# gregorgebhardt/gym-kilobots

Measured on AMD Instinct MI355X. Metric: kilobot-steps/sec, higher is better.
Workload: dtype f32

## Files before the change

### gym_kilobots_amd/csrc/kb_common.h

```cpp
#pragma once
#include <hip/hip_runtime.h>

#include <cmath>
#include <cstdio>
#include <cstring>
#include <type_traits>

#include "kilobots_hip.h"
#include "kb_launch.h"
#include "kb_exact.h"

namespace kb {

constexpr float B2_PI = 3.14159265359f;
constexpr float B2_LINEAR_SLOP = 0.005f;
constexpr float B2_POLYGON_RADIUS = 2.0f * B2_LINEAR_SLOP;
constexpr float B2_BAUMGARTE = 0.2f;
constexpr float B2_MAX_LINEAR_CORRECTION = 0.2f;
constexpr float B2_MAX_TRANSLATION = 2.0f;
constexpr float B2_MAX_TRANSLATION_SQ = B2_MAX_TRANSLATION * B2_MAX_TRANSLATION;
constexpr float B2_MAX_ROTATION = 0.5f * B2_PI;
constexpr float B2_MAX_ROTATION_SQ = B2_MAX_ROTATION * B2_MAX_ROTATION;
constexpr float B2_EPSILON = 1.19209290e-07f;
constexpr float B2_TOI_BAUMGARTE = 0.75f;
constexpr int B2_MAX_SUBSTEPS = 8;
constexpr float B2_TIME_TO_SLEEP = 0.5f;
constexpr float B2_LINEAR_SLEEP_TOL = 0.01f;
constexpr float B2_ANGULAR_SLEEP_TOL = 2.0f / 180.0f * B2_PI;
constexpr float WORLD_SCALE = 25.0f;

constexpr float CELL_SIZE = 0.875f;
constexpr int MAX_CELLS = 8192;

constexpr unsigned KEY_WALL = 0x10000u, KEY_OBJ = 0x20000u;
constexpr int WALL_CODE = 0xFFF0;
constexpr int OBJ_CODE = 0xFFE0;
constexpr int MAXOBJ = KB_MAX_OBJECTS;
constexpr unsigned short EMPTY16 = 0xFFFFu;

#ifndef KB_KREG
#define KB_KREG 2
#endif
constexpr int MAX_BUCKETS = MAX_WAVES * BK_PER_WAVE;
constexpr int GIANT_ISLAND = 256;
constexpr int BIG_ISLAND = 16;
constexpr int KREG = KB_KREG;
#ifndef KB_NSOLVE_DIV
#define KB_NSOLVE_DIV 1
#endif
#ifndef KB_KREG_BINS
#define KB_KREG_BINS (2 * KB_NSOLVE_DIV)
#endif

enum { M_NCON = 0, M_TOTAL = 1, M_ANY = 2, M_STATUS = 3, M_MAXISL = 4, M_PROF = 5, M_XTRA = 6, M_XFILL = 7, M_WCNT = 8, M_WAKE = 32 , M_WFILL = 8 + MAX_WAVES, M_COUNT = 8 + 2 * MAX_WAVES };
static_assert(M_COUNT <= 64, "misc area");

struct Params {
    kb_buffers buf;
    const float *actions;
    const float *light_action;
    int N, NP, NB, M, E, S, gw, gh, ncell, cap, capL, n_substeps, flags, drive_mode, light_type, vel_iters, pos_iters;
    int solver_mode, toi_walls;
    float xmin, ymin, xmax, ymax, inv_cell, r_bot, im_bot, kl_bot, ka_bot, h;
    float light_radius, light_lo[2], light_hi[2], act_lo[2], act_hi[2];
    int lcount, ladim, lkind[KB_MAX_LIGHTS];
    float lradius[KB_MAX_LIGHTS], lmaxv[KB_MAX_LIGHTS];
    float llo[KB_MAX_LIGHTS][2], lhi[KB_MAX_LIGHTS][2], lalo[KB_MAX_LIGHTS][2], lahi[KB_MAX_LIGHTS][2];
    float kl_obj, ka_obj;
    float otab[KB_MAX_OBJECTS][OT_WORDS_C];
    float obody[KB_MAX_OBJECTS][BT_WORDS_C];
    int F;
    float mu_oo, mu_ow;
    int nmc;
    int lds_total;
    int nhead, hmask;
    int allow_sleep;
    float im_mode[5];
    int botlaw_off;
    int islmin_off;
    int sense_s;
    float sense_r2;
    float rr2, rw2, rw_tot;
    float toi_tt;
    float nm_bb, nm_wb;
    float y_bb, y_wb;
    int exact_div;
    const unsigned char *env_mask;
};


__device__ __forceinline__ void kb_sincosf(float xx, float &sn, float &cs) {
    const float DP1 = 0.78515625f, DP2 = 2.4187564849853515625e-4f, DP3 = 3.77489497744594108e-8f;
    const float FOPI = 1.27323954473516f;
    float x = fabsf(xx);
    int j = (int)(FOPI * x);
    float y = (float)j;
    if (j & 1) { j += 1; y += 1.0f; }
    j &= 7;
    float ssign = xx < 0.0f ? -1.0f : 1.0f, csign = 1.0f;
    if (j > 3) { ssign = -ssign; csign = -csign; j -= 4; }
    if (j > 1) csign = -csign;
    x = ((x - y * DP1) - y * DP2) - y * DP3;
    float z = x * x;
    float pc = ((2.443315711809948E-005f * z - 1.388731625493765E-003f) * z + 4.166664568298827E-002f) * z * z
               - 0.5f * z + 1.0f;
    float ps = ((-1.9515295891E-4f * z + 8.3321608736E-3f) * z - 1.6666654611E-1f) * z * x + x;
    if (j == 1 || j == 2) { sn = ssign * pc; cs = csign * ps; }
    else { sn = ssign * ps; cs = csign * pc; }
}

__device__ __forceinline__ void kb_light_circular(float sx, float sy, float lx, float ly, float R,
                                                  float &val, float &gx, float &gy) {
    float dx = -1.0f * (sx - lx), dy = -1.0f * (sy - ly);
    float n = sqrtf(dx * dx + dy * dy);
    float v = 1.0f - n / R;
    v = fmaxf(fminf(v, 1.0f), 0.0f);
    val = v * 255.0f;
    if (n > 0.0f) { dx = dx / n; dy = dy / n; }
    else { dx = 0.0f; dy = 0.0f; }
    if (n > R) { dx *= 0.0f; dy *= 0.0f; }
    gx = dx; gy = dy;
}

__device__ __forceinline__ void kb_light_single_step(const Params &p, const float *la, float h, float &lx, float &ly) {
    float ax = fminf(fmaxf(la[0], p.act_lo[0]), p.act_hi[0]);
    float ay = fminf(fmaxf(la[1], p.act_lo[1]), p.act_hi[1]);
    float nlx = lx + ax * h, nly = ly + ay * h;
    lx = fminf(fmaxf(nlx, p.light_lo[0]), p.light_hi[0]);
    ly = fminf(fmaxf(nly, p.light_lo[1]), p.light_hi[1]);
}
__device__ __forceinline__ void kb_light_general_step(const Params &p, const float *la, float h, float (&glx)[KB_MAX_LIGHTS],
                                                      float (&gly)[KB_MAX_LIGHTS], float (&glvx)[KB_MAX_LIGHTS], float (&glvy)[KB_MAX_LIGHTS]) {
    if (p.light_type == KB_LIGHT_GRADIENT) {
        const float pi = 3.14159265358979323846f;
        float ang = fminf(fmaxf(la[0], -2.0f * pi), 2.0f * pi);
        if (ang < -pi) ang += 2.0f * pi;
        if (ang > pi) ang -= 2.0f * pi;
        glx[0] = ang;
    } else {
#pragma unroll
        for (int i = 0; i < KB_MAX_LIGHTS; ++i) {
            if (i >= p.lcount) break;
            const float ax = fminf(fmaxf(la[2 * i + 0], p.lalo[i][0]), p.lahi[i][0]);
            const float ay = fminf(fmaxf(la[2 * i + 1], p.lalo[i][1]), p.lahi[i][1]);
            float nlx, nly;
            if (p.lkind[i] == KB_LIGHT_MOMENTUM) {
                float mvx = glvx[i] + ax * h, mvy = glvy[i] + ay * h;
                const float nv = sqrtf(mvx * mvx + mvy * mvy);
                if (nv > p.lmaxv[i]) { const float sc = p.lmaxv[i] / nv; mvx *= sc; mvy *= sc; }
                glvx[i] = mvx; glvy[i] = mvy;
                nlx = glx[i] + mvx * h; nly = gly[i] + mvy * h;
            } else {
                nlx = glx[i] + ax * h; nly = gly[i] + ay * h;
            }
            glx[i] = fminf(fmaxf(nlx, p.llo[i][0]), p.lhi[i][0]);
            gly[i] = fminf(fmaxf(nly, p.llo[i][1]), p.lhi[i][1]);
        }
    }
}
__device__ __forceinline__ void kb_light_general_sense(const Params &p, const float (&glx)[KB_MAX_LIGHTS], const float (&gly)[KB_MAX_LIGHTS],
                                                       float sx, float sy, float &val, float &gx, float &gy) {
    if (p.light_type == KB_LIGHT_GRADIENT) {
        float s_, c_;
        kb_sincosf(glx[0], s_, c_);
        val = c_ * sx + s_ * sy; gx = c_; gy = s_;
        return;
    }
    float vsum = 0.0f, vbest = 0.0f, bgx = 0.0f, bgy = 0.0f;
#pragma unroll
    for (int i = 0; i < KB_MAX_LIGHTS; ++i) {
        if (i >= p.lcount) break;
        float v, x, y;
        kb_light_circular(sx, sy, glx[i], gly[i], p.lradius[i], v, x, y);
        vsum = i == 0 ? v : vsum + v;
        if (i == 0 || v > vbest) { vbest = v; bgx = x; bgy = y; }
    }
    val = vsum; gx = bgx; gy = bgy;
}

__device__ __forceinline__ void kb_motor_law(int ml, int mr, float th, float h, float &vx, float &vy, float &w) {
    const float max_lin = 0.01f, max_ang = 0.5f * 3.14159265358979323846f;
    float s, c;
    kb_sincosf(th, s, c);
    if (ml && mr) {
        float lin = (float)(mr + ml) / 510.0f * max_lin;
        vx = (s * lin) * WORLD_SCALE; vy = (c * lin) * WORLD_SCALE;
        w = (float)(mr - ml) / 510.0f * max_ang;
    } else if (mr || ml) {
        float av, lx, ly = -0.009f;
        if (mr) { av = (float)mr / 255.0f * max_ang; lx = -0.013f; }
        else { av = -(float)ml / 255.0f * max_ang; lx = 0.013f; }
        float ds, dc;
        kb_sincosf(av * h, ds, dc);
        float tx = lx - (dc * lx - ds * ly), ty = ly - (ds * lx + dc * ly);
        tx *= WORLD_SCALE; ty *= WORLD_SCALE;
        float wx = c * tx - s * ty, wy = s * tx + c * ty;
        wx = wx / WORLD_SCALE / h; wy = wy / WORLD_SCALE / h;
        vx = wx * WORLD_SCALE; vy = wy * WORLD_SCALE; w = av;
    } else {
        vx = 0.0f; vy = 0.0f; w = 0.0f;
    }
}

__device__ __forceinline__ float kb_clampf(float a, float lo, float hi) { return fmaxf(lo, fminf(a, hi)); }

__device__ __forceinline__ void wave_sync() {
    __builtin_amdgcn_fence(__ATOMIC_RELEASE, "wavefront");
    __builtin_amdgcn_wave_barrier();
    __builtin_amdgcn_fence(__ATOMIC_ACQUIRE, "wavefront");
}

template <bool DS_ATOMIC = false>
__device__ __forceinline__ unsigned lds_load_relaxed(const unsigned *p_) {
    if constexpr (DS_ATOMIC) return atomicOr(const_cast<unsigned *>(p_), 0u);
    else return *reinterpret_cast<const volatile unsigned *>(p_);
}

__device__ __forceinline__ void lds_barrier() {
    asm volatile("s_waitcnt lgkmcnt(0)\n\ts_barrier" ::: "memory");
}

#define KB_DPP(v, ctrl, rows) __builtin_amdgcn_update_dpp(0, (int)(v), ctrl, rows, 0xf, true)
__device__ __forceinline__ unsigned wave_or(unsigned v) {
    v |= (unsigned)KB_DPP(v, 0x111, 0xf);
    v |= (unsigned)KB_DPP(v, 0x112, 0xf);
    v |= (unsigned)KB_DPP(v, 0x114, 0xf);
    v |= (unsigned)KB_DPP(v, 0x118, 0xf);
    v |= (unsigned)KB_DPP(v, 0x142, 0xa);
    v |= (unsigned)KB_DPP(v, 0x143, 0xc);
    return (unsigned)__builtin_amdgcn_readlane((int)v, 63);
}
__device__ __forceinline__ unsigned wave_umax(unsigned v) {
    v = max(v, (unsigned)KB_DPP(v, 0x111, 0xf));
    v = max(v, (unsigned)KB_DPP(v, 0x112, 0xf));
    v = max(v, (unsigned)KB_DPP(v, 0x114, 0xf));
    v = max(v, (unsigned)KB_DPP(v, 0x118, 0xf));
    v = max(v, (unsigned)KB_DPP(v, 0x142, 0xa));
    v = max(v, (unsigned)KB_DPP(v, 0x143, 0xc));
    return (unsigned)__builtin_amdgcn_readlane((int)v, 63);
}
__device__ __forceinline__ unsigned wave_incl_scan(unsigned v) {
// ... 347 lines not shown
```

### gym_kilobots_amd/csrc/kb_step_kernel.h

```cpp
#pragma once
#include <utility>

#include "kb_common.h"
#include "kb_objects.h"

namespace kb {

template <int DRIVE_MODE, int LIGHT_TYPE, bool OBJ, int FN = 0, int TIER = 0, bool POLY = true, bool SENSE = true, bool SLEEP = false>
__global__ void __launch_bounds__(TIER == 1 ? 64 : 64 * KB_MAX_WAVES, (TIER == 1 || TIER == 3) ? 2 : ((TIER == 2 || (FN != 0 && !OBJ)) ? KB_COMPACT_WAVES_PER_SIMD : KB_MIN_WAVES_PER_SIMD)) kb_step_kernel(const Params p) {
    constexpr bool WIDE = TIER == 1 || TIER == 3;
    constexpr bool BINS = !OBJ;
    constexpr int KRX = BINS ? KB_KREG_BINS : KREG;
    constexpr bool PAR_DS = FN != 0 && BINS;
    static_assert(!SLEEP || FN == 0 || !OBJ, "the fixed-size instantiations with objects do not carry the sleep state");
    extern __shared__ __align__(16) unsigned char smem[];
    {
        static_assert(sizeof(Params) >= 6 * 64, "the six lines asked for are kernel arguments");
        const __attribute__((address_space(4))) unsigned *ka_ = (const __attribute__((address_space(4))) unsigned *)__builtin_amdgcn_kernarg_segment_ptr();
        const __attribute__((address_space(1))) unsigned char *m_ = (const __attribute__((address_space(1))) unsigned char *)p.env_mask;
        asm volatile("" : "+s"(m_) : "s"(ka_[0]), "s"(ka_[16]), "s"(ka_[32]), "s"(ka_[48]), "s"(ka_[64]), "s"(ka_[80]));
        if (m_ && !m_[blockIdx.x]) return;
    }
    int e = blockIdx.x;
    int tid = threadIdx.x;
    const int nt = FN ? 64 * KB_MAX_WAVES : (int)blockDim.x;
    int lane = tid & 63, wave = tid >> 6;
    const int wave_s = __builtin_amdgcn_readfirstlane(wave);
    const int nw = nt >> 6;
    const int nsolve = BINS ? (nw >= KB_NSOLVE_DIV ? nw / KB_NSOLVE_DIV : 1) : nw;
    const int N = FN ? FN : p.N, NP = FN ? ((FN + 3) & ~3) : p.NP, S = p.S;
    size_t o = (size_t)e * N;
    size_t wo = (size_t)e * p.cap;
    const float h = p.h;

    const int NB = FN ? ((FN + 3) & ~3) + KB_MAX_OBJECTS + 4 : p.NB;
    const int capL_ = (BINS && FN != 0) ? ldsb::CAPL : p.capL;
    const bool hashed = FN == 0 && p.hmask != 0;
    const int fx = lds::fixed(OBJ || FN != 0, nw), ot_ = lds::objtab(nw);
    float2 *pos = (float2 *)(smem + (BINS ? ldsb::pos() : lds::body32(fx, NB, 0))), *vel = (float2 *)(smem + (BINS ? ldsb::vel(NB) : lds::body32(fx, NB, 2)));
    float2 *start = (float2 *)(smem + lds::body32(fx, NB, 4));
    unsigned *dirCnt = (unsigned *)(smem + (BINS ? ldsb::dircnt(NB) : lds::body32(fx, NB, 6))), *parent = (unsigned *)(smem + (BINS ? ldsb::parent(NB) : lds::body32(fx, NB, 7)));
    unsigned *islCnt = dirCnt;
    unsigned *lPair = (unsigned *)(smem + (BINS ? ldsb::con32(NB, NP, hashed, capL_, 0) : lds::con32(fx, NB, capL_, 0))), *lInfo = (unsigned *)(smem + (BINS ? ldsb::con32(NB, NP, hashed, capL_, 1) : lds::con32(fx, NB, capL_, 1)));
    float *lAcc = (float *)(smem + (BINS ? ldsb::con32(NB, NP, hashed, capL_, 2) : lds::con32(fx, NB, capL_, 2)));
    float *oldAcc = (float *)(smem + (BINS ? ldsb::oldacc(NB, NP, hashed, capL_) : lds::con32(fx, NB, capL_, 3)));
    unsigned short *lCbk = (unsigned short *)(smem + (BINS ? ldsb::cbk(NB, NP, hashed, capL_) : lds::con16(fx, NB, capL_, 0)));
    unsigned short *lOrder = (unsigned short *)(smem + (BINS ? ldsb::order(NB, NP, hashed, capL_) : lds::con16(fx, NB, capL_, 1)));
    unsigned short *oldKey = (unsigned short *)(smem + (BINS ? ldsb::oldkey(NB, NP, hashed, capL_) : lds::con16(fx, NB, capL_, 2)));
    unsigned short *wsOff = (unsigned short *)(smem + (BINS ? ldsb::wsoff(NB) : lds::bot16(fx, NB, capL_, NP, 0))), *newOff = (unsigned short *)(smem + (BINS ? ldsb::newoff(NB, NP, hashed) : lds::bot16(fx, NB, capL_, NP, 1)));
    unsigned short *nextb = (unsigned short *)(smem + lds::bot16(fx, NB, capL_, NP, 2)), *cellOf = (unsigned short *)(smem + lds::bot16(fx, NB, capL_, NP, 3));
    unsigned char *wsCnt = smem + (BINS ? ldsb::wscnt(NB, NP) : lds::bot8(fx, NB, capL_, NP, 0)), *wsCntNew = smem + (BINS ? ldsb::wscntnew(NB, NP, hashed) : lds::bot8(fx, NB, capL_, NP, 1));
    unsigned char *active = smem + (BINS ? ldsb::act0(NB, NP, hashed, capL_) : lds::active(fx, NB, capL_, NP));
    unsigned char *islWave = smem + (BINS ? ldsb::islwave(NB, NP, hashed, capL_) : lds::islwave(fx, NB, capL_, NP));
    unsigned short *head = (unsigned short *)(smem + lds::head(fx, NB, capL_, NP));
    unsigned short *idOf = (unsigned short *)(smem + ldsb::idof(NB, NP)), *cellOfSlot = (unsigned short *)(smem + ldsb::cellofslot(NB, NP));
    unsigned short *E1 = (unsigned short *)(smem + ldsb::binE(NB, NP, hashed, capL_));
    unsigned short *tmpSort = reinterpret_cast<unsigned short *>(lInfo);
    float *startX = reinterpret_cast<float *>(smem + ldsb::botA(NB)), *startY = reinterpret_cast<float *>(dirCnt);
    unsigned *misc = (unsigned *)(smem + lds::MISC), *wsum = (unsigned *)(smem + lds::WSUM);
    const int tb_ = BINS ? ldsb::binE(NB, NP, hashed, capL_) - lds::BKSTART : 0;
    unsigned *bkStart = (unsigned *)(smem + tb_ + lds::BKSTART), *bkFill = (unsigned *)(smem + tb_ + lds::bkfill(nw));
    unsigned *bkMaxRank = (unsigned *)(smem + tb_ + lds::bkmaxrank(nw));
    unsigned short *bkList = (unsigned short *)(smem + tb_ + lds::bklist(nw));
    unsigned char *nList = smem + tb_ + lds::nlist(nw);
    unsigned *intMark = reinterpret_cast<unsigned *>(bkList);
    static_assert(BPT * 64 * KB_MAX_WAVES <= 1024 && lds::nbk(1) >= 64, "32 words of intMark hold a bit for every slot");
    float *objTab = (float *)(smem + ot_);
    float *objBody = (float *)(smem + ot_ + lds::OBJBODY);
    unsigned *objCnt = (unsigned *)(smem + ot_ + lds::OBJCNT);
    unsigned short *objList = (unsigned short *)(smem + ot_ + lds::OBJLIST);
    float *objW = (float *)(smem + ot_ + lds::OBJW), *objA = (float *)(smem + ot_ + lds::OBJA), *objA0 = (float *)(smem + ot_ + lds::OBJA0);
    unsigned long long *mcMask = (unsigned long long *)(smem + ot_ + lds::MCMASK);
    float *objSlp = (float *)(smem + ot_ + lds::OBJSLP);
    const int M = OBJ ? p.M : 0;
    constexpr bool MIX = DRIVE_MODE == KB_DRIVE_MIXED;
    static_assert(!MIX || (OBJ && FN == 0), "mixed drive laws run on the generic code path with per-body masses");
    unsigned char *botLaw = smem + (MIX ? p.botlaw_off : 0);
#define KB_IM_BOT(a_) (MIX ? p.im_mode[botLaw[a_]] : p.im_bot)
    auto bim = [&](int id) __attribute__((always_inline)) -> float {
        return id >= WALL_CODE ? 0.0f : ((!OBJ || id < N) ? KB_IM_BOT(id) : objBody[(id - N) * BT_WORDS + BT_IM]);
    };
    auto brad = [&](int id) __attribute__((always_inline)) -> float {
        return id >= WALL_CODE ? B2_POLYGON_RADIUS : ((!OBJ || id < N) ? p.r_bot : objBody[(id - N) * BT_WORDS + BT_RADIUS]);
    };
    auto bpoly = [&](int id) __attribute__((always_inline)) -> bool {
        return OBJ && POLY && id >= N && id < WALL_CODE && objBody[(id - N) * BT_WORDS + BT_KIND] != 0.0f;
    };
    ObjCtx ox;
    ox.pos = pos; ox.vel = vel; ox.objW = objW; ox.objA = objA; ox.objTab = objTab; ox.objBody = objBody;
    ox.mc = (float *)(smem + lds::mcarea(fx, NB, capL_, NP, p.nhead));
    ox.N = N; ox.MCN = p.nmc; ox.mu_oo = p.mu_oo; ox.mu_ow = p.mu_ow;
    const int NMC = OBJ ? p.nmc : 0;
    const int F = OBJ ? p.F : 0;

    const kb_buffers &g = p.buf;
    auto hix = [&](int cell_) __attribute__((always_inline)) -> int { return hashed ? (cell_ & p.hmask) : cell_; };
    unsigned *gPair, *gInfo;
    float *gAcc;
    unsigned short *gCbk, *gOrder;
#define KB_ENV_ADDRESSES()                                                                          \
    do {                                                                                            \
        int e_ = blockIdx.x;                                                                        \
        asm volatile("" : "+s"(e_));                                                                \
        e = e_; o = (size_t)e * N; wo = (size_t)e * p.cap;                                          \
        gPair = reinterpret_cast<unsigned *>(g.scratch) + wo * 4;                                   \
        gInfo = gPair + p.cap;                                                                      \
        gAcc = reinterpret_cast<float *>(gInfo + p.cap);                                            \
        gCbk = reinterpret_cast<unsigned short *>(gAcc + p.cap); gOrder = gCbk + p.cap;             \
    } while (0)
    KB_ENV_ADDRESSES();

#ifdef KB_PROFILE
    static_assert(M_COUNT <= 24, "profile words start at misc[24]");
    constexpr int M_PROF_DEPTH = 12;
    if (tid < 40) misc[24 + tid] = 0;
    __syncthreads();
    unsigned prof_t = (unsigned)clock64();
#endif

    float th[BPT], bw[BPT], cv[BPT], cw[BPT], av[BPT], aw[BPT];
    float sth0[BPT];
    float slp[BPT];
    int law[BPT];
    int ms[BPT];
#define KB_LAW(q) (MIX ? law[q] : DRIVE_MODE)
    constexpr bool PARK = BINS && !MIX && DRIVE_MODE == KB_DRIVE_VELOCITY;
#define KB_SLOT(q, b_) (BINS ? ms[q] : (b_))
    float ldx[BPT], ldy[BPT];
    unsigned ldc[BPT];
    float2 lda[BPT];
#pragma unroll
    for (int q = 0; q < BPT; ++q) {
        const int b = tid + q * nt;
        th[q] = 0.0f; bw[q] = 0.0f; cv[q] = 0.0f; cw[q] = 0.0f; av[q] = 0.0f; aw[q] = 0.0f; slp[q] = 0.0f; law[q] = DRIVE_MODE;
        float z_ = 0.0f;
        asm volatile("" : "+v"(z_));
        ldx[q] = 0.0f; ldy[q] = 0.0f; ldc[q] = 0u; lda[q] = make_float2(z_, z_);
        ms[q] = b < N ? b : NB - 1;
        if (b < N) {
            ldx[q] = g.x[o + b]; ldy[q] = g.y[o + b]; th[q] = g.theta[o + b];
            if (MIX) law[q] = min((int)g.bot_mode[o + b], 4);
            if (SLEEP) slp[q] = g.sleep_time[o + b];
            ldc[q] = g.ws_cnt[o + b];
            const bool velmode = KB_LAW(q) == KB_DRIVE_VELOCITY || KB_LAW(q) == KB_DRIVE_ACCEL;
            if (velmode && !(KB_LAW(q) == KB_DRIVE_VELOCITY && p.actions)) { cv[q] = g.v[o + b]; cw[q] = g.w[o + b]; }
            if (KB_LAW(q) == KB_DRIVE_ACCEL) { av[q] = g.acc_v[o + b]; aw[q] = g.acc_w[o + b]; }
            if (p.actions && velmode) lda[q] = reinterpret_cast<const float2 *>(p.actions)[o + b];
        }
    }
    unsigned pfKey[2] = {0u, 0u};
    float pfAcc[2] = {0.0f, 0.0f};
    if (BINS && p.n_substeps > 0) {
#pragma unroll
        for (int q = 0; q < 2; ++q) {
            const int i = tid + q * nt;
            if (i < capL_ && i < p.cap) { pfKey[q] = g.ws_key[wo + i]; pfAcc[q] = g.ws_acc[wo + i]; }
        }
    }
    int hasAct = __builtin_amdgcn_readfirstlane((int)(p.actions != nullptr));
    asm volatile("" : "+s"(hasAct));
#pragma unroll
    for (int q = 0; q < BPT; ++q) {
        const int b = tid + q * nt;
        if (b < N) {
            pos[b] = make_float2(ldx[q], ldy[q]);
            if (MIX) botLaw[b] = (unsigned char)law[q];
            wsCnt[b] = (unsigned char)ldc[q];
            if (hasAct) {
                const float2 a = lda[q];
                const float mw = 0.5f * 3.14159265358979323846f;
                if (KB_LAW(q) == KB_DRIVE_VELOCITY) {
                    cv[q] = fmaxf(fminf(a.x, 0.01f), 0.0f);
                    cw[q] = fmaxf(fminf(a.y, mw), -mw);
                    g.v[o + b] = cv[q]; g.w[o + b] = cw[q];
                } else if (KB_LAW(q) == KB_DRIVE_ACCEL) {
                    const float aw_ = 0.2f * 3.14159265358979323846f;
                    av[q] = fmaxf(fminf(a.x, 0.005f), -0.005f);
                    aw[q] = fmaxf(fminf(a.y, aw_), -aw_);
                    g.acc_v[o + b] = av[q]; g.acc_w[o + b] = aw[q];
                }
            }
            if (PARK) vel[b] = make_float2(cv[q], cw[q]);
        }
    }
    for (int b = N + tid; b < NP; b += nt) { wsCnt[b] = 0; wsCntNew[b] = 0; }
    if (tid < M) {
        const size_t oi = (size_t)e * M + tid;
        pos[N + tid].x = g.ox[oi]; pos[N + tid].y = g.oy[oi]; vel[N + tid].x = g.ovx[oi]; vel[N + tid].y = g.ovy[oi];
        objA[tid] = g.otheta[oi]; objW[tid] = g.ow[oi];
        if (SLEEP) objSlp[tid] = g.osleep[oi];
        const float lx = p.obody[tid][BT_LCX], ly = p.obody[tid][BT_LCY];
        if (lx != 0.0f || ly != 0.0f) {
            const XF t = xf_make(g.ox[oi], g.oy[oi], g.otheta[oi]);
            const V2 cm = xf_mul(t, mk2(lx, ly));
            pos[N + tid].x = cm.x; pos[N + tid].y = cm.y;
        }
    }
    for (int k = tid; k < F * OT_WORDS; k += nt) objTab[k] = p.otab[k / OT_WORDS][k % OT_WORDS];
    for (int k = tid; k < M * BT_WORDS; k += nt) objBody[k] = p.obody[k / BT_WORDS][k % BT_WORDS];
    bool mcTouch = false;
    float *owsMine = nullptr;
    if (BINS) { for (int c = tid; c < ldsb::bin_entries(p.nhead) / 2; c += nt) reinterpret_cast<unsigned *>(E1)[c] = 0u; }
    else for (int c = tid; c < p.nhead; c += nt) head[c] = EMPTY16;
    if (tid == 0) misc[M_STATUS] = 0;
    float lx = 0.0f, ly = 0.0f;
    if (LIGHT_TYPE == KB_LIGHT_CIRCULAR) { lx = g.light_x[e]; ly = g.light_y[e]; }
    constexpr bool LGEN = LIGHT_TYPE == KB_LIGHT_GENERAL;
    float glx[KB_MAX_LIGHTS], gly[KB_MAX_LIGHTS], glvx[KB_MAX_LIGHTS], glvy[KB_MAX_LIGHTS];
#pragma unroll
    for (int i = 0; i < KB_MAX_LIGHTS; ++i) {
        glx[i] = 0.0f; gly[i] = 0.0f; glvx[i] = 0.0f; glvy[i] = 0.0f;
        if (LGEN && i < p.lcount) {
            glx[i] = g.light_x[(size_t)e * p.lcount + i];
            if (p.light_type != KB_LIGHT_GRADIENT) gly[i] = g.light_y[(size_t)e * p.lcount + i];
            if (p.lkind[i] == KB_LIGHT_MOMENTUM) { glvx[i] = g.light_vx[(size_t)e * p.lcount + i]; glvy[i] = g.light_vy[(size_t)e * p.lcount + i]; }
        }
    }
    auto sense_general = [&](float sx, float sy, float &val, float &gx, float &gy) __attribute__((always_inline)) {
        kb_light_general_sense(p, glx, gly, sx, sy, val, gx, gy);
    };
    const bool drive = !(p.flags & KB_STEP_NO_DRIVE);
    const float rr2 = p.rr2, rw2 = p.rw2;
    __syncthreads();
    unsigned oldTotal = block_scan_u8(wsCnt, wsOff, NP, wsum, tid);
    bool oldInLds = oldTotal <= (unsigned)capL_;
    if (BINS && oldInLds) {
#pragma unroll
        for (int q = 0; q < 2; ++q) {
            const unsigned i = tid + q * nt;
            if (i < oldTotal) {
                oldKey[i] = (unsigned short)(pfKey[q] >= KEY_WALL ? WALL_CODE + (pfKey[q] - KEY_WALL) : pfKey[q]);
                oldAcc[i] = pfAcc[q];
            }
        }
    }
    if (oldInLds) {
        for (unsigned i = tid + (BINS ? 2 * nt : 0); i < oldTotal; i += nt) {
            const unsigned k = g.ws_key[wo + i];
            oldKey[i] = (unsigned short)(k >= KEY_OBJ ? OBJ_CODE + (k - KEY_OBJ) : (k >= KEY_WALL ? WALL_CODE + (k - KEY_WALL) : k));
            oldAcc[i] = g.ws_acc[wo + i];
        }
    }
    __syncthreads();

    KB_STAMP(13);
    for (int sub = 0; sub < p.n_substeps; ++sub) {
        KB_ENV_ADDRESSES();
#ifdef KB_ABLATE
#define KB_ABLATE_EXIT(k_) do { if (KB_ABLATE == (k_)) return; } while (0)
#else
#define KB_ABLATE_EXIT(k_) do { } while (0)
#endif
#define KB_RETID() do { int w_ = __builtin_amdgcn_readfirstlane(wave_s); asm volatile("" : "+s"(w_));                                                                  \
                        int l_ = (int)__builtin_amdgcn_mbcnt_hi(~0u, __builtin_amdgcn_mbcnt_lo(~0u, 0u)); asm volatile("" : "+v"(l_));    \
                        wave = w_; lane = l_; tid = (w_ << 6) | l_; } while (0)
        KB_RETID();
        if (p.light_action && LGEN && drive)
            kb_light_general_step(p, p.light_action + (size_t)e * p.ladim, h, glx, gly, glvx, glvy);
        if (p.light_action && LIGHT_TYPE == KB_LIGHT_CIRCULAR && drive)
            kb_light_single_step(p, p.light_action + 2 * e, h, lx, ly);
        float sbx[BPT], sby[BPT], svx[BPT], svy[BPT];
        int scell[BPT], sarr[BPT];
#define SC_CX(s_) ((s_) & 0xFFF)
#define SC_CY(s_) (((s_) >> 12) & 0xFFF)
#pragma unroll
        for (int q = 0; q < BPT; ++q) {
            const int b = tid + q * nt;
            sbx[q] = 0.0f; sby[q] = 0.0f; svx[q] = 0.0f; svy[q] = 0.0f; scell[q] = 0; sarr[q] = 0;
            if (b >= N) continue;
            float bvx = 0.0f, bvy = 0.0f, bww = 0.0f;
            const float bx = pos[KB_SLOT(q, b)].x, by = pos[KB_SLOT(q, b)].y;
            if (!BINS) { start[b].x = bx; start[b].y = by; }
            sth0[q] = th[q];
            if (drive) {
                const float t = th[q];
                float lval = 0.0f, lgx = 0.0f, lgy = 0.0f;
                if (LIGHT_TYPE != KB_LIGHT_NONE) {
                    float sx = bx, sy = by;
                    if (KB_LAW(q) != KB_DRIVE_SIMPLE_PHOTOTAXIS) {
                        float s, c;
                        kb_sincosf(t, s, c);
                        const float lx0 = 0.0f, ly0 = -p.r_bot;
                        sx = (c * lx0 - s * ly0) + bx;
                        sy = (s * lx0 + c * ly0) + by;
                    }
                    if (LGEN) sense_general(sx / WORLD_SCALE, sy / WORLD_SCALE, lval, lgx, lgy);
                    else kb_light_circular(sx / WORLD_SCALE, sy / WORLD_SCALE, lx, ly, p.light_radius, lval, lgx, lgy);
                    if (g.light_value) { g.light_value[o + b] = lval; g.light_gx[o + b] = lgx; g.light_gy[o + b] = lgy; }
                }
                switch (KB_LAW(q)) {
                case KB_DRIVE_ACCEL: {
                    float v = cv[q] + av[q] * h, ww = cw[q] + aw[q] * h;
                    const float mw = 0.5f * 3.14159265358979323846f;
                    v = fminf(fmaxf(v, 0.0f), 0.01f); ww = fminf(fmaxf(ww, -mw), mw);
                    cv[q] = v; cw[q] = ww;
                    float s, c;
                    kb_sincosf(t, s, c);
                    float sp = v * WORLD_SCALE;
                    bvx = c * sp; bvy = s * sp; bww = ww;
                } break;
                case KB_DRIVE_VELOCITY: {
                    float s, c;
                    kb_sincosf(t, s, c);
                    float cvq = cv[q], cwq = cw[q];
                    if (PARK) { const float2 c_ = vel[b]; cvq = c_.x; cwq = c_.y; }
                    asm volatile("" : "+v"(cvq));
                    float sp = cvq * WORLD_SCALE;
                    bvx = c * sp; bvy = s * sp; bww = cwq;
                } break;
                case KB_DRIVE_PHOTOTAXIS: {
                    int upd = g.pt_update[o + b];
                    if (upd % 6 == 0) {
                        float meas = lval;
                        if (meas > g.pt_threshold[o + b] || g.pt_nochange[o + b] >= 15) {
                            g.pt_threshold[o + b] = meas + 0.01f;
                            if (g.pt_dir[o + b] == 0) { g.pt_dir[o + b] = 1; g.motor_l[o + b] = 0; g.motor_r[o + b] = 255; }
                            else { g.pt_dir[o + b] = 0; g.motor_l[o + b] = 255; g.motor_r[o + b] = 0; }
                            g.pt_nochange[o + b] = 0;
                        } else g.pt_nochange[o + b] += 1;
                    }
                    g.pt_update[o + b] = upd + 1;
                    kb_motor_law(g.motor_l[o + b], g.motor_r[o + b], t, h, bvx, bvy, bww);
                } break;
                case KB_DRIVE_MOTORS:
                    kb_motor_law(g.motor_l[o + b], g.motor_r[o + b], t, h, bvx, bvy, bww);
                    break;
                case KB_DRIVE_SIMPLE_PHOTOTAXIS: {
                    float n = sqrtf(lgx * lgx + lgy * lgy);
                    float mx = lgx, my = lgy;
                    if (n > 0.01f) { mx = lgx / n * 0.01f; my = lgy / n * 0.01f; }
                    bvx = mx * WORLD_SCALE; bvy = my * WORLD_SCALE; bww = 0.0f;
                } break;
                default: break;
                }
            }
            if (g.cmd_vx) { g.cmd_vx[o + b] = bvx; g.cmd_vy[o + b] = bvy; g.cmd_w[o + b] = bww; }
            if (SLEEP) {
                if (drive && slp[q] < 0.0f && (bww * bww > 0.0f || bvx * bvx + bvy * bvy > 0.0f)) slp[q] = 0.0f;
                if (slp[q] < 0.0f) { bvx = 0.0f; bvy = 0.0f; bww = 0.0f; }
                active[b] = 0;
            }
            const float kl = (KB_LAW(q) == KB_DRIVE_SIMPLE_PHOTOTAXIS) ? 1.0f / (1.0f + h * 0.0f) : p.kl_bot;
            bw[q] = bww * p.ka_bot;
            int cx = (int)floorf((bx - p.xmin) * p.inv_cell);
            int cy = (int)floorf((by - p.ymin) * p.inv_cell);
            cx = cx < 0 ? 0 : (cx >= p.gw ? p.gw - 1 : cx);
            cy = cy < 0 ? 0 : (cy >= p.gh ? p.gh - 1 : cy);
            const int cell = cy * p.gw + cx;
            if (BINS) {
                sbx[q] = bx; sby[q] = by; svx[q] = bvx * kl; svy[q] = bvy * kl; scell[q] = cx | (cy << 12);
                const int bi = (hashed ? (cell & p.hmask) : cell) + 1;
                const unsigned old = atomicAdd(reinterpret_cast<unsigned *>(E1) + (bi >> 1), 1u << (16 * (bi & 1)));
                sarr[q] = (int)((old >> (16 * (bi & 1))) & 0xFFFFu);
                if (SENSE && p.sense_s > 0) reinterpret_cast<unsigned short *>(lAcc)[b] = 0;
            } else {
                vel[b].x = bvx * kl; vel[b].y = bvy * kl;
                parent[b] = b;
                cellOf[b] = (unsigned short)cell;
                nextb[b] = (unsigned short)kb_exch16(head, hix(cell), (unsigned)b);
                if (SENSE && p.sense_s > 0) newOff[b] = 0;
            }
        }
        if (tid < M) { start[N + tid].x = pos[N + tid].x; start[N + tid].y = pos[N + tid].y; objA0[tid] = objA[tid]; }
        if (tid < M) {
            vel[N + tid].x *= p.kl_obj; vel[N + tid].y *= p.kl_obj; objW[tid] *= p.ka_obj;
            parent[N + tid] = N + tid;
            objCnt[tid] = 0;
            if (SLEEP) active[N + tid] = 0;
        }
        if (OBJ && tid >= M && tid < F) objCnt[tid] = 0;
        if (tid < M_COUNT && tid != M_STATUS) misc[tid] = 0;
        if (SLEEP && tid < 32) misc[M_WAKE + tid] = 0;
        KB_STAMP_PRE(16);
        __syncthreads();
        KB_STAMP(0);
        KB_RETID();
        KB_ABLATE_EXIT(1);
        auto ws_find = [&](int owner, unsigned key16) __attribute__((always_inline)) -> float {
            const int cnt = wsCnt[owner], off = wsOff[owner];
            if (oldInLds) {
                for (int s = 0; s < cnt; ++s)
                    if (oldKey[off + s] == (unsigned short)key16) {
                        const float a_ = oldAcc[off + s];
                        if (SLEEP) oldAcc[off + s] = -1.0f - a_;
                        return a_;
                    }
            } else {
                const unsigned key32 = key16 >= (unsigned)WALL_CODE ? KEY_WALL + (key16 - WALL_CODE)
                                     : (key16 >= (unsigned)OBJ_CODE ? KEY_OBJ + (key16 - OBJ_CODE) : key16);
                for (int s0 = 0; s0 < cnt; s0 += 4) {
                    unsigned k4[4];
#pragma unroll
                    for (int u = 0; u < 4; ++u) {
                        const int idx = off + s0 + u;
                        k4[u] = (s0 + u < cnt && idx < p.cap) ? g.ws_key[wo + idx] : 0xFFFFFFFFu;
                    }
#pragma unroll
                    for (int u = 0; u < 4; ++u)
                        if (k4[u] == key32) {
                            const float a_ = g.ws_acc[wo + off + s0 + u];
                            if (SLEEP) g.ws_acc[wo + off + s0 + u] = -1.0f - a_;
                            return a_;
                        }
                }
            }
            return -1.0f;
        };
        bool big = false;
        int stageCap = 0, ncon = 0;
        unsigned newTotal = 0;
        if constexpr (BINS) {
            {
                const int nchunks = ldsb::bin_entries(p.nhead) >> 3;
                if (nchunks <= nt) block_scan_bins<true>(E1, nchunks, 1, wsum, tid);
                else block_scan_bins<false>(E1, nchunks, (nchunks + nt - 1) / nt, wsum, tid);
            }
            KB_STAMP_PRE(31);
#pragma unroll
            for (int q = 0; q < BPT; ++q) {
                const int b = tid + q * nt;
                if (b >= N) continue;
                const int cell = SC_CY(scell[q]) * p.gw + SC_CX(scell[q]);
                const int bin = hashed ? (cell & p.hmask) : cell;
                tmpSort[(int)E1[bin] + sarr[q]] = (unsigned short)b;
            }
            __syncthreads();
            KB_STAMP_PRE(32);
            KB_RETID();
#pragma unroll
            for (int q = 0; q < BPT; ++q) {
                const int b = tid + q * nt;
                if (b >= N) continue;
                const int cell = SC_CY(scell[q]) * p.gw + SC_CX(scell[q]);
                const int bin = hashed ? (cell & p.hmask) : cell;
                const int s0 = (int)E1[bin], s1 = (int)E1[bin + 1];
                int rank = 0;
                if (s1 - s0 > 1)
                    for (int s_ = s0; s_ < s1; ++s_) rank += ((int)tmpSort[s_] < b) ? 1 : 0;
                const int sl = s0 + rank;
                ms[q] = sl;
                idOf[sl] = (unsigned short)b;
                if (hashed) cellOfSlot[sl] = (unsigned short)cell;
                pos[sl] = make_float2(sbx[q], sby[q]);
                vel[sl] = make_float2(svx[q], svy[q]);
                parent[sl] = (unsigned)sl;
            }
            if (tid < 4) {
                float z_ = 0.0f;
                asm volatile("" : "+v"(z_));
                vel[NB - 5 + tid] = make_float2(z_, z_);
            }
            KB_STAMP_PRE(33);
            __syncthreads();
            KB_STAMP(0);
            KB_RETID();
            KB_ABLATE_EXIT(2);
            if (SENSE && p.sense_s > 0 && drive) {
#pragma unroll 1
                for (int q = 0; q < BPT; ++q) {
                    const int b = tid + q * nt;
                    if (b >= N) continue;
                    const int sl = q == 0 ? ms[0] : ms[BPT - 1];
                    const int sc = q == 0 ? scell[0] : scell[BPT - 1];
                    if (hashed) kb_sense_bins_hashed(pos, E1, cellOfSlot, reinterpret_cast<unsigned *>(lAcc), sl, SC_CX(sc), SC_CY(sc), p.gw, p.gh, p.sense_s, p.sense_r2, p.hmask);
                    else kb_sense_bins(pos, E1, reinterpret_cast<unsigned *>(lAcc), sl, SC_CX(sc), SC_CY(sc), p.gw, p.gh, p.sense_s, p.sense_r2);
                }
            }
            constexpr int NR = FN ? 3 : 5;
            auto candidate_runs = [&](int sa, int cx, int cy, int (&lo)[NR], int (&hi)[NR], int (&sp)[NR], int (&tc)[5]) __attribute__((always_inline)) {
                const int gw = p.gw, gh = p.gh;
                const int cell = cy * gw + cx;
                const bool e_ok = cx + 1 < gw, n_ok = cy + 1 < gh, w_ok = cx > 0;
                tc[0] = cell; tc[1] = cell + 1; tc[2] = cell + gw; tc[3] = cell + gw + 1; tc[4] = cell + gw - 1;
                if constexpr (NR == 3) {
                    const int up = cell + gw;
                    const int e1 = (int)E1[cell + 1], e2 = (int)E1[e_ok ? cell + 2 : cell + 1];
                    const int u0 = (int)E1[n_ok ? (w_ok ? up - 1 : up) : 0], u1 = (int)E1[n_ok ? up : 0];
                    const int u2 = (int)E1[n_ok ? up + 1 : 0], u3 = (int)E1[n_ok ? (e_ok ? up + 2 : up + 1) : 0];
                    lo[0] = sa + 1; sp[0] = e1; hi[0] = e2;
                    lo[1] = u1; sp[1] = u2; hi[1] = u3;
                    lo[2] = u0; sp[2] = u1; hi[2] = u1;
                } else {
                    const bool ok[5] = {true, e_ok, n_ok, n_ok && e_ok, n_ok && w_ok};
#pragma unroll
                    for (int k = 0; k < 5; ++k) {
                        const int bin = hashed ? (tc[k] & p.hmask) : tc[k];
                        const int l_ = ok[k] ? (int)E1[bin] : 0, h_ = ok[k] ? (int)E1[bin + 1] : 0;
                        lo[k] = k == 0 ? sa + 1 : l_; hi[k] = h_; sp[k] = h_;
                    }
                }
            };
            auto for_partners = [&](int sa, int cx, int cy, auto &&cb) __attribute__((always_inline)) {
                int lo[NR], hi[NR], sp[NR], tc[5];
                candidate_runs(sa, cx, cy, lo, hi, sp, tc);
                int pre[NR + 1];
                pre[0] = 0;
#pragma unroll
                for (int r = 0; r < NR; ++r) pre[r + 1] = pre[r] + max(hi[r] - lo[r], 0);
                const int tot = pre[NR];
                const float2 pa = pos[sa];
#ifndef KB_FIND_BATCH
#define KB_FIND_BATCH 2
#endif
                constexpr int BATCH = KB_FIND_BATCH;
                for (int base = 0; base < tot; base += BATCH) {
                    int cs[BATCH], ck[BATCH];
                    float2 cp[BATCH];
                    int cc[BATCH];
#pragma unroll
                    for (int u = 0; u < BATCH; ++u) {
                        const int i = base + u;
                        int sl = lo[0] + i, spl = sp[0], kb_ = 0;
#pragma unroll
                        for (int r = 1; r < NR; ++r)
                            if (i >= pre[r]) { sl = lo[r] + (i - pre[r]); spl = sp[r]; kb_ = NR == 3 ? 2 * r : r; }
                        ck[u] = kb_ + ((NR == 3 && sl >= spl) ? 1 : 0);
                        cs[u] = i < tot ? sl : sa;
// ... 1876 lines not shown
```

Before: 17.28 billion.

## Reorder kernel-arg layout and restructure prologue loads to shorten startup latency

Moves hot Params fields into a contiguous prefix and touches one dword per hot kernarg line (plus a trailing word) so they are scalar-loaded early. It also hoists the warm-start prefetch ahead of the per-bot loads, selects the command source pointer uniformly so one load path serves both action and stored-velocity cases, and loads the circular light position through the constant address space earlier. Object-only init is gated on OBJ at compile time. The aim is to cut prologue latency in a short kernel, at the cost of more complex and fragile argument-layout assumptions.

```diff
diff --git a/gym_kilobots_amd/csrc/kb_common.h b/gym_kilobots_amd/csrc/kb_common.h
--- a/gym_kilobots_amd/csrc/kb_common.h
+++ b/gym_kilobots_amd/csrc/kb_common.h
@@ -2,6 +2,7 @@
 #include <hip/hip_runtime.h>
 
 #include <cmath>
+#include <cstddef>
 #include <cstdio>
 #include <cstring>
 #include <type_traits>
@@ -59,9 +60,21 @@
     kb_buffers buf;
     const float *actions;
     const float *light_action;
+    const unsigned char *env_mask;
     int N, NP, NB, M, E, S, gw, gh, ncell, cap, capL, n_substeps, flags, drive_mode, light_type, vel_iters, pos_iters;
     int solver_mode, toi_walls;
     float xmin, ymin, xmax, ymax, inv_cell, r_bot, im_bot, kl_bot, ka_bot, h;
+    int nhead, hmask;
+    int lds_total;
+    int allow_sleep;
+    int islmin_off;
+    int sense_s;
+    float sense_r2;
+    float rr2, rw2, rw_tot;
+    float toi_tt;
+    float nm_bb, nm_wb;
+    float y_bb, y_wb;
+    int exact_div;
     float light_radius, light_lo[2], light_hi[2], act_lo[2], act_hi[2];
     int lcount, ladim, lkind[KB_MAX_LIGHTS];
     float lradius[KB_MAX_LIGHTS], lmaxv[KB_MAX_LIGHTS];
@@ -72,21 +85,13 @@
     int F;
     float mu_oo, mu_ow;
     int nmc;
-    int lds_total;
-    int nhead, hmask;
-    int allow_sleep;
     float im_mode[5];
     int botlaw_off;
-    int islmin_off;
-    int sense_s;
-    float sense_r2;
-    float rr2, rw2, rw_tot;
-    float toi_tt;
-    float nm_bb, nm_wb;
-    float y_bb, y_wb;
-    int exact_div;
-    const unsigned char *env_mask;
 };
+constexpr int KB_ARG_LINE = 64, KB_HOT_ARG_LINES = 9;
+static_assert(offsetof(Params, buf) == 0 && offsetof(Params, act_hi) + sizeof(Params::act_hi) <= KB_HOT_ARG_LINES * KB_ARG_LINE &&
+              offsetof(Params, act_hi) + sizeof(Params::act_hi) > (KB_HOT_ARG_LINES - 1) * KB_ARG_LINE, "the hot prefix of Params is KB_HOT_ARG_LINES lines");
+static_assert(offsetof(Params, lcount) >= offsetof(Params, act_hi) + sizeof(Params::act_hi), "the fields read on demand lie behind the hot prefix");
 
 
 __device__ __forceinline__ void kb_sincosf(float xx, float &sn, float &cs) {
diff --git a/gym_kilobots_amd/csrc/kb_step_kernel.h b/gym_kilobots_amd/csrc/kb_step_kernel.h
--- a/gym_kilobots_amd/csrc/kb_step_kernel.h
+++ b/gym_kilobots_amd/csrc/kb_step_kernel.h
@@ -15,10 +15,13 @@
     static_assert(!SLEEP || FN == 0 || !OBJ, "the fixed-size instantiations with objects do not carry the sleep state");
     extern __shared__ __align__(16) unsigned char smem[];
     {
-        static_assert(sizeof(Params) >= 6 * 64, "the six lines asked for are kernel arguments");
+        static_assert(KB_HOT_ARG_LINES == 9 && sizeof(Params) >= KB_HOT_ARG_LINES * KB_ARG_LINE, "one dword of every line of the hot prefix is asked for");
+        constexpr int LW = KB_ARG_LINE / 4;
+        constexpr int GSX = ((int)sizeof(Params) + 7) / 8 * 8 + 12;
         const __attribute__((address_space(4))) unsigned *ka_ = (const __attribute__((address_space(4))) unsigned *)__builtin_amdgcn_kernarg_segment_ptr();
         const __attribute__((address_space(1))) unsigned char *m_ = (const __attribute__((address_space(1))) unsigned char *)p.env_mask;
-        asm volatile("" : "+s"(m_) : "s"(ka_[0]), "s"(ka_[16]), "s"(ka_[32]), "s"(ka_[48]), "s"(ka_[64]), "s"(ka_[80]));
+        asm volatile("" : "+s"(m_) : "s"(ka_[0]), "s"(ka_[LW]), "s"(ka_[2 * LW]), "s"(ka_[3 * LW]), "s"(ka_[4 * LW]), "s"(ka_[5 * LW]), "s"(ka_[6 * LW]),
+                                     "s"(ka_[7 * LW]), "s"(ka_[8 * LW]), "s"(ka_[GSX / 4]));
         if (m_ && !m_[blockIdx.x]) return;
     }
     int e = blockIdx.x;
@@ -126,35 +129,66 @@
 #define KB_LAW(q) (MIX ? law[q] : DRIVE_MODE)
     constexpr bool PARK = BINS && !MIX && DRIVE_MODE == KB_DRIVE_VELOCITY;
 #define KB_SLOT(q, b_) (BINS ? ms[q] : (b_))
+    unsigned pfKey[2] = {0u, 0u};
+    float pfAcc[2] = {0.0f, 0.0f};
+    if (BINS && p.n_substeps > 0) {
+#pragma unroll
+        for (int q = 0; q < 2; ++q) {
+            const int i = tid + q * nt;
+            if (i < capL_ && i < p.cap) { pfKey[q] = g.ws_key[wo + i]; pfAcc[q] = g.ws_acc[wo + i]; }
+        }
+    }
     float ldx[BPT], ldy[BPT];
     unsigned ldc[BPT];
-    float2 lda[BPT];
+    float ldc0[BPT], ldc1[BPT];
+    float ldv[BPT], ldw[BPT];
+    int hasActL = __builtin_amdgcn_readfirstlane((int)(p.actions != nullptr));
+    asm volatile("" : "+s"(hasActL));
+    constexpr bool SELCMD = !MIX && (DRIVE_MODE == KB_DRIVE_VELOCITY || DRIVE_MODE == KB_DRIVE_ACCEL);
+    const float *stored0 = DRIVE_MODE == KB_DRIVE_ACCEL ? g.acc_v : g.v, *stored1 = DRIVE_MODE == KB_DRIVE_ACCEL ? g.acc_w : g.w;
+    const char *cmd0 = hasActL ? reinterpret_cast<const char *>(p.actions) : reinterpret_cast<const char *>(stored0);
+    const char *cmd1 = hasActL ? reinterpret_cast<const char *>(p.actions + 1) : reinterpret_cast<const char *>(stored1);
+    const int cmdShift = hasActL ? 3 : 2;
 #pragma unroll
     for (int q = 0; q < BPT; ++q) {
         const int b = tid + q * nt;
         th[q] = 0.0f; bw[q] = 0.0f; cv[q] = 0.0f; cw[q] = 0.0f; av[q] = 0.0f; aw[q] = 0.0f; slp[q] = 0.0f; law[q] = DRIVE_MODE;
-        float z_ = 0.0f;
-        asm volatile("" : "+v"(z_));
-        ldx[q] = 0.0f; ldy[q] = 0.0f; ldc[q] = 0u; lda[q] = make_float2(z_, z_);
+        ldx[q] = 0.0f; ldy[q] = 0.0f; ldc[q] = 0u; ldc0[q] = 0.0f; ldc1[q] = 0.0f; ldv[q] = 0.0f; ldw[q] = 0.0f;
         ms[q] = b < N ? b : NB - 1;
         if (b < N) {
             ldx[q] = g.x[o + b]; ldy[q] = g.y[o + b]; th[q] = g.theta[o + b];
             if (MIX) law[q] = min((int)g.bot_mode[o + b], 4);
             if (SLEEP) slp[q] = g.sleep_time[o + b];
             ldc[q] = g.ws_cnt[o + b];
-            const bool velmode = KB_LAW(q) == KB_DRIVE_VELOCITY || KB_LAW(q) == KB_DRIVE_ACCEL;
-            if (velmode && !(KB_LAW(q) == KB_DRIVE_VELOCITY && p.actions)) { cv[q] = g.v[o + b]; cw[q] = g.w[o + b]; }
-            if (KB_LAW(q) == KB_DRIVE_ACCEL) { av[q] = g.acc_v[o + b]; aw[q] = g.acc_w[o + b]; }
-            if (p.actions && velmode) lda[q] = reinterpret_cast<const float2 *>(p.actions)[o + b];
+            if (SELCMD) {
+                ldc0[q] = *reinterpret_cast<const float *>(cmd0 + ((o + b) << cmdShift));
+                ldc1[q] = *reinterpret_cast<const float *>(cmd1 + ((o + b) << cmdShift));
+            }
+            if (KB_LAW(q) == KB_DRIVE_ACCEL) {
+                ldv[q] = g.v[o + b]; ldw[q] = g.w[o + b];
+                if (!SELCMD) { av[q] = g.acc_v[o + b]; aw[q] = g.acc_w[o + b]; }
+            }
         }
     }
-    unsigned pfKey[2] = {0u, 0u};
-    float pfAcc[2] = {0.0f, 0.0f};
-    if (BINS && p.n_substeps > 0) {
-#pragma unroll
-        for (int q = 0; q < 2; ++q) {
-            const int i = tid + q * nt;
-            if (i < capL_ && i < p.cap) { pfKey[q] = g.ws_key[wo + i]; pfAcc[q] = g.ws_acc[wo + i]; }
+    float lx = 0.0f, ly = 0.0f;
+    if (LIGHT_TYPE == KB_LIGHT_CIRCULAR) {
+        typedef const __attribute__((address_space(4))) float *cfloat_p;
+        lx = *(cfloat_p)(g.light_x + e); ly = *(cfloat_p)(g.light_y + e);
+    }
+    if (!SELCMD && hasActL) {
+#pragma unroll
+        for (int q = 0; q < BPT; ++q) {
+            const int b = tid + q * nt;
+            if (b < N && (KB_LAW(q) == KB_DRIVE_VELOCITY || KB_LAW(q) == KB_DRIVE_ACCEL)) {
+                const float2 a = reinterpret_cast<const float2 *>(p.actions)[o + b];
+                ldc0[q] = a.x; ldc1[q] = a.y;
+            }
+        }
+    } else if (!SELCMD) {
+#pragma unroll
+        for (int q = 0; q < BPT; ++q) {
+            const int b = tid + q * nt;
+            if (b < N && KB_LAW(q) == KB_DRIVE_VELOCITY) { ldc0[q] = g.v[o + b]; ldc1[q] = g.w[o + b]; }
         }
     }
     int hasAct = __builtin_amdgcn_readfirstlane((int)(p.actions != nullptr));
@@ -167,21 +201,23 @@
             if (MIX) botLaw[b] = (unsigned char)law[q];
             wsCnt[b] = (unsigned char)ldc[q];
             if (hasAct) {
-                const float2 a = lda[q];
                 const float mw = 0.5f * 3.14159265358979323846f;
                 if (KB_LAW(q) == KB_DRIVE_VELOCITY) {
-                    cv[q] = fmaxf(fminf(a.x, 0.01f), 0.0f);
-                    cw[q] = fmaxf(fminf(a.y, mw), -mw);
+                    cv[q] = fmaxf(fminf(ldc0[q], 0.01f), 0.0f);
+                    cw[q] = fmaxf(fminf(ldc1[q], mw), -mw);
                     g.v[o + b] = cv[q]; g.w[o + b] = cw[q];
                 } else if (KB_LAW(q) == KB_DRIVE_ACCEL) {
                     const float aw_ = 0.2f * 3.14159265358979323846f;
-                    av[q] = fmaxf(fminf(a.x, 0.005f), -0.005f);
-                    aw[q] = fmaxf(fminf(a.y, aw_), -aw_);
+                    av[q] = fmaxf(fminf(ldc0[q], 0.005f), -0.005f);
+                    aw[q] = fmaxf(fminf(ldc1[q], aw_), -aw_);
                     g.acc_v[o + b] = av[q]; g.acc_w[o + b] = aw[q];
                 }
-            }
+            } else if (KB_LAW(q) == KB_DRIVE_VELOCITY) { cv[q] = ldc0[q]; cw[q] = ldc1[q]; }
+            else if (SELCMD && KB_LAW(q) == KB_DRIVE_ACCEL) { av[q] = ldc0[q]; aw[q] = ldc1[q]; }
             if (PARK) vel[b] = make_float2(cv[q], cw[q]);
         }
+        if (SELCMD && DRIVE_MODE == KB_DRIVE_ACCEL) asm volatile("v_mov_b32 %0, %2\n\tv_mov_b32 %1, %3" : "=&v"(cv[q]), "=&v"(cw[q]) : "v"(ldv[q]), "v"(ldw[q]));
+        else if (MIX && law[q] == KB_DRIVE_ACCEL) { cv[q] = ldv[q]; cw[q] = ldw[q]; }
     }
     for (int b = N + tid; b < NP; b += nt) { wsCnt[b] = 0; wsCntNew[b] = 0; }
     if (tid < M) {
@@ -203,8 +239,6 @@
     if (BINS) { for (int c = tid; c < ldsb::bin_entries(p.nhead) / 2; c += nt) reinterpret_cast<unsigned *>(E1)[c] = 0u; }
     else for (int c = tid; c < p.nhead; c += nt) head[c] = EMPTY16;
     if (tid == 0) misc[M_STATUS] = 0;
-    float lx = 0.0f, ly = 0.0f;
-    if (LIGHT_TYPE == KB_LIGHT_CIRCULAR) { lx = g.light_x[e]; ly = g.light_y[e]; }
     constexpr bool LGEN = LIGHT_TYPE == KB_LIGHT_GENERAL;
     float glx[KB_MAX_LIGHTS], gly[KB_MAX_LIGHTS], glvx[KB_MAX_LIGHTS], glvy[KB_MAX_LIGHTS];
 #pragma unroll
@@ -361,8 +395,8 @@
                 if (SENSE && p.sense_s > 0) newOff[b] = 0;
             }
         }
-        if (tid < M) { start[N + tid].x = pos[N + tid].x; start[N + tid].y = pos[N + tid].y; objA0[tid] = objA[tid]; }
-        if (tid < M) {
+        if (OBJ && tid < M) { start[N + tid].x = pos[N + tid].x; start[N + tid].y = pos[N + tid].y; objA0[tid] = objA[tid]; }
+        if (OBJ && tid < M) {
             vel[N + tid].x *= p.kl_obj; vel[N + tid].y *= p.kl_obj; objW[tid] *= p.ka_obj;
             parent[N + tid] = N + tid;
             objCnt[tid] = 0;
```

Measured after the change: 17.27 billion. About the same (-0.0%).
